# GuanLab/seekmer

Hardware: AMD Instinct MI355X
Metric: paired reads/sec mapped+quantified (higher is better)
Workload: dtype u64+f64; 1 GPU; configs[1]: synthetic ~190k-tx index (stand-in for ENSEMBL GRCh38 cDNA), 10000000 2x100bp synthetic pairs per GPU, map+classes+EM to the reference stop rule; transcripts=190402, kmer_slots=134217728, units_per_gpu=10000000, read_len=100, paired=True, classes=851072, class_map_rows=4208693, parallelism=reads sharded x1, RCCL all-reduce f64[T] per EM step, rccl_ranks=0

## Files before the change

include/seekmer_hip.h:

```cpp
#ifndef SEEKMER_HIP_H
#define SEEKMER_HIP_H

#include <stddef.h>
#include <stdint.h>

#ifdef __cplusplus
extern "C" {
#endif

#define SKM_OK 0
#define SKM_ERR_ARG 1
#define SKM_ERR_HIP 2
#define SKM_ERR_NO_DEVICE 3
#define SKM_ERR_COLLISION 4
#define SKM_ERR_STATE 5
#define SKM_ERR_IO 6
#define SKM_ERR_UNDEFINED 7
#define SKM_ERR_COMM 8

#define SKM_KMER_SIZE 25
#define SKM_MAX_FRAGMENT_LENGTH 2000


const char *skm_last_error(void);
// ... 194 lines not shown
                               int64_t n_tx, double *out);
int skm_effective_lengths_weights(int device, int64_t n, const double *p, const double *lengths,
                                  int64_t n_tx, double *out);

int skm_bias_correct(skm_index *index, int strand, const int64_t *observed, const double *tpm, const double *eff,
                     int64_t n_tx, double *expected_out, double *b_out, double *eff_out);
int skm_bias_correct_many(skm_index *index, int strand, int64_t n, const int64_t *observed, const double *tpm,
                          const double *eff, int64_t n_tx, double *expected_out, double *b_out, double *eff_out);
int skm_bias_fixed_weights(const double *tpm, const int32_t *windows, int64_t n_tx, uint64_t *limbs_out,
                           double *total_out);

typedef struct skm_quant skm_quant;
int skm_quant_create(int device, int64_t n_tx, int64_t n_classes,
                     const int64_t *class_offsets, const int32_t *class_targets,
                     const double *class_counts, skm_quant **out);
int skm_quant_create_from_mapper(skm_mapper *mapper, int64_t n_tx, skm_quant **out);
int skm_quant_destroy(skm_quant *quant);
int skm_quant_em(skm_quant *quant, double *x, const double *l, double rel_tol,
                 double x_floor, int64_t max_iters, int64_t fixed_iters,
                 int64_t *iters);
int skm_quant_bootstrap(skm_quant *quant, int64_t n_boot, uint64_t seed,
                        const double *x0, const double *l, double rel_tol,
                        double x_floor, int64_t max_iters, double *out,
                        int64_t *counts_out, int64_t *iters_out);
int skm_quant_bootstrap_tpm(skm_quant *quant, int64_t n_boot, uint64_t seed,
                            const double *x0, const double *l, double rel_tol,
                            double x_floor, int64_t max_iters, double *out,
                            int64_t *iters_out);
int skm_quant_bootstrap_share_tpm(skm_quant *quant, int64_t n_boot, int64_t first, int64_t step,
                                  uint64_t seed, const double *x0, const double *l, double rel_tol,
                                  double x_floor, int64_t max_iters, double *out,
                                  int64_t *iters_out);
int skm_quant_set_counts(skm_quant *quant, const double *class_counts);
int skm_quant_em_many(skm_quant *quant, int64_t n_sets, const double *counts, const double *x0,
                      const double *l, double rel_tol, double x_floor, int tpm, double *out,
                      int64_t *iters_out);
int skm_quant_em_blend(skm_quant *quant, int64_t n_cells, const int32_t *class_cell,
                       const double *weight, const double *cell_total, const double *x0,
                       const double *l, double rel_tol, double x_floor, int tpm, double *out,
                       int64_t *iters_out, double *counts_out);
int skm_quant_em_tables(int device, int64_t n_tx, int64_t n_tables, const int64_t *table_class_offsets,
                        const int64_t *class_offsets, const int32_t *class_targets,
                        const double *class_counts, const double *x0, const double *l, double rel_tol,
                        double x_floor, int64_t max_iters, int tpm, double *out, int64_t *iters);
int skm_set_quant_groups(int64_t n_tables, int64_t n_tx, const int64_t *table_classes,
                         const int64_t *table_ids, int64_t max_slots, int64_t *n_groups,
                         int64_t *group_first);
int skm_sample_set_quantify(skm_sample_set *set, const double *lengths, int64_t n_tx, double rel_tol,
                            double x_floor, int64_t max_iters, int64_t cap_samples,
                            int64_t *n_samples, double *tpm, double *effective_lengths,
                            int64_t *iters);
int skm_quant_components(skm_quant *quant, int64_t info[8], int32_t *tx_label, int32_t *tx_tile,
                         int32_t *class_tile);
int skm_quant_timing(skm_quant *quant, double timing[4]);

typedef struct skm_comm skm_comm;
int skm_comm_unique_id(void *id128);
int skm_comm_create(int device, const void *id128, int rank, int world, skm_comm **out);
int skm_comm_count(skm_comm *comm, int *count);
int skm_comm_destroy(skm_comm *comm);
int skm_mapper_exchange_tables(skm_mapper *send, int send_to, skm_mapper *recv, int recv_from, skm_comm *comm);
int skm_quant_set_comm(skm_quant *quant, skm_comm *comm);

int skm_quant_infer(skm_mapper *mapper, skm_comm *comm, const double *lengths, int64_t n_tx,
                    double rel_tol, double x_floor, int64_t max_iters,
                    double *tpm, double *effective_lengths, int64_t *iters);


typedef struct skm_built skm_built;
int skm_build_index(const char *pool, const int64_t *seq_offsets, int64_t n_seqs,
                    int n_threads, skm_built **out);
int skm_built_sizes(const skm_built *b, int64_t sizes[4]);
int skm_built_copy(const skm_built *b, void *kmers, void *contigs,
                   char *sequences, void *targets);
int skm_built_free(skm_built *b);

typedef struct skm_fastq skm_fastq;
int skm_fastq_open(const char *const *paths, int n_paths, int paired,
                   int64_t batch_units, skm_fastq **out);
int skm_fastq_set_allocator(skm_fastq *reader, void *(*alloc)(size_t), void (*release)(void *));
int skm_fastq_set_parallel(skm_fastq *reader, int n_threads, int *enabled);
int skm_fastq_set_shard(skm_fastq *reader, int rank, int world);
int skm_fastq_batch_index(const skm_fastq *reader, int64_t *index);
int skm_fastq_batch_read_length(const skm_fastq *reader, int64_t *read_len);
int skm_fastq_next(skm_fastq *reader, int64_t *n_units, const char **bases,
                   const int64_t **offsets, const char **names,
                   const int64_t **name_offsets);
typedef struct skm_fastq_slab skm_fastq_slab;
int skm_fastq_detach(skm_fastq *reader, skm_fastq_slab **slab);
int skm_fastq_recycle(skm_fastq *reader, skm_fastq_slab *slab);
int skm_fastq_close(skm_fastq *reader);

int skm_fastq_cache_bytes(int64_t bytes);
int skm_fastq_wait_unmapped(void);
typedef struct skm_fastq_prefault skm_fastq_prefault;
int skm_fastq_prefault_start(const char *const *paths, int n_paths, int n_threads, skm_fastq_prefault **out);
int skm_fastq_prefault_finish(skm_fastq_prefault *handle);

typedef struct skm_fastq_packed skm_fastq_packed;
int skm_fastq_packed_open(const char *const *paths, int n_paths, int paired, int n_threads,
                          int64_t chunk_bytes, int want_names, skm_fastq_packed **out);
int skm_fastq_packed_open_ranges(const char *const *paths, int n_paths, int paired, int n_threads,
                                 int64_t chunk_bytes, int want_names, const int64_t *begin,
                                 const int64_t *end, int64_t first_unit, skm_fastq_packed **out);
int skm_fastq_count_newlines(const char *path, int64_t chunk_bytes, int64_t first_chunk,
                             int64_t chunk_step, int n_threads, int64_t *counts, int64_t n_chunks,
// ... 35 lines not shown
```

seekmer_amd/_native.py:

```python
import ctypes
import os

_HERE = os.path.dirname(os.path.abspath(__file__))
HIP_LIB_PATH = os.environ.get('SKM_HIP_LIB') or os.path.join(_HERE, 'libseekmer_hip.so')
HOST_LIB_PATH = os.path.join(_HERE, 'libseekmer_host.so')

SKM_OK = 0
SKM_ERR_ARG = 1
SKM_ERR_HIP = 2
SKM_ERR_NO_DEVICE = 3
SKM_ERR_COLLISION = 4
SKM_ERR_STATE = 5
SKM_ERR_IO = 6
SKM_ERR_UNDEFINED = 7
SKM_ERR_COMM = 8

SKM_STRAND_NONE = 0
SKM_STRAND_FR = 1
SKM_STRAND_RF = 2

c_void_pp = ctypes.POINTER(ctypes.c_void_p)
c_i64p = ctypes.POINTER(ctypes.c_int64)
c_i32p = ctypes.POINTER(ctypes.c_int32)
c_f64p = ctypes.POINTER(ctypes.c_double)
# ... 115 lines not shown
                                       c_i64p]),
    'skm_sample_set_plan': (ctypes.c_int, [c_i64, c_i32p, c_i64p, c_i64, c_i64, c_i64p, c_i64p, c_i64p, c_i32p]),
    'skm_sample_set_split': (ctypes.c_int, [c_i64, c_i64p, c_i64p, c_i32p, c_i64, c_i64, c_i64p, c_i32p, c_i64p, c_i64p,
                                            c_i64p]),
    'skm_gene_sums': (ctypes.c_int, [ctypes.c_int, c_i64, c_i64, c_i64, c_i32p, c_f64p, c_f64p]),
    'skm_gene_unique_counts': (ctypes.c_int, [ctypes.c_int, c_i64, c_i64p, c_i32p, c_i64p, c_i32p, c_i64, c_i64, c_i64,
                                              c_i32p, c_i64p, c_i64p]),
    'skm_mapper_gene_counts': (ctypes.c_int, [ctypes.c_void_p, c_i64, c_i64, c_i32p, c_i64p, c_i64p]),
    'skm_sample_set_gene_counts': (ctypes.c_int, [ctypes.c_void_p, c_i64, c_i64, c_i32p, c_i64, c_i64p, c_i64p]),
    'skm_sample_set_gene_matrix': (ctypes.c_int, [ctypes.c_void_p, c_i64, c_i64, c_i32p, c_void_pp]),
    'skm_gene_matrix_from_classes': (ctypes.c_int, [ctypes.c_int, c_i64, c_i64p, c_i32p, c_i64p, c_i32p, c_i64, c_i64, c_i64,
                                                    c_i32p, c_void_pp]),
    'skm_gene_matrix_shape': (ctypes.c_int, [ctypes.c_void_p, c_i64p, c_i64p, c_i64p]),
    'skm_gene_matrix_read': (ctypes.c_int, [ctypes.c_void_p, c_i64p, c_i32p, c_i64p, c_i64p]),
    'skm_gene_matrix_destroy': (ctypes.c_int, [ctypes.c_void_p]),
    'skm_barcodes_create':(ctypes.c_int, [ctypes.c_int, ctypes.c_char_p, c_i64, ctypes.c_int, c_void_pp]),
    'skm_barcodes_destroy': (ctypes.c_int, [ctypes.c_void_p]),
    'skm_barcodes_assign': (ctypes.c_int, [ctypes.c_void_p, ctypes.POINTER(PackedReads), ctypes.c_int, ctypes.c_int,
                                           c_i32p, c_i64p, c_i64p]),
    'skm_units_group': (ctypes.c_int, [ctypes.c_int, c_i32p, c_i64, c_i64, c_i32p, c_i64p]),
    'skm_barcode_census_create': (ctypes.c_int, [ctypes.c_int, ctypes.c_int, c_void_pp]),
    'skm_barcode_census_destroy': (ctypes.c_int, [ctypes.c_void_p]),
    'skm_barcode_census_add': (ctypes.c_int, [ctypes.c_void_p, ctypes.POINTER(PackedReads), ctypes.c_int, c_i64p]),
    'skm_barcode_census_size': (ctypes.c_int, [ctypes.c_void_p, c_i64p, c_i64p]),
    'skm_barcode_census_ranked': (ctypes.c_int, [ctypes.c_void_p, c_i64, c_u64p, c_i64p]),
    'skm_barcode_census_pick': (ctypes.c_int, [ctypes.c_void_p, c_i64, ctypes.c_int, c_i64, c_u64p, c_i64p, c_i64p]),
    'skm_quant_create': (ctypes.c_int, [ctypes.c_int, c_i64, c_i64, c_i64p, c_i32p, c_f64p,
                                        c_void_pp]),
    'skm_quant_create_from_mapper': (ctypes.c_int, [ctypes.c_void_p, c_i64, c_void_pp]),
    'skm_quant_destroy': (ctypes.c_int, [ctypes.c_void_p]),
    'skm_quant_em': (ctypes.c_int, [ctypes.c_void_p, c_f64p, c_f64p, ctypes.c_double,
                                    ctypes.c_double, c_i64, c_i64, c_i64p]),
    'skm_quant_bootstrap': (ctypes.c_int, [ctypes.c_void_p, c_i64, ctypes.c_uint64, c_f64p,
                                           c_f64p, ctypes.c_double, ctypes.c_double, c_i64,
                                           c_f64p, c_i64p, c_i64p]),
    'skm_quant_bootstrap_tpm': (ctypes.c_int, [ctypes.c_void_p, c_i64, ctypes.c_uint64, c_f64p,
                                               c_f64p, ctypes.c_double, ctypes.c_double, c_i64,
                                               c_f64p, c_i64p]),
    'skm_quant_bootstrap_share_tpm': (ctypes.c_int, [ctypes.c_void_p, c_i64, c_i64, c_i64, ctypes.c_uint64, c_f64p,
                                                     c_f64p, ctypes.c_double, ctypes.c_double, c_i64,
                                                     c_f64p, c_i64p]),
    'skm_quant_set_counts': (ctypes.c_int, [ctypes.c_void_p, c_f64p]),
    'skm_quant_em_many': (ctypes.c_int, [ctypes.c_void_p, c_i64, c_f64p, c_f64p, c_f64p, ctypes.c_double,
                                         ctypes.c_double, ctypes.c_int, c_f64p, c_i64p]),
    'skm_quant_em_blend': (ctypes.c_int, [ctypes.c_void_p, c_i64, c_i32p, c_f64p, c_f64p, c_f64p, c_f64p,
                                          ctypes.c_double, ctypes.c_double, ctypes.c_int, c_f64p, c_i64p, c_f64p]),
    'skm_quant_em_tables': (ctypes.c_int, [ctypes.c_int, c_i64, c_i64, c_i64p, c_i64p, c_i32p, c_f64p, c_f64p, c_f64p,
                                           ctypes.c_double, ctypes.c_double, c_i64, ctypes.c_int, c_f64p, c_i64p]),
    'skm_set_quant_groups': (ctypes.c_int, [c_i64, c_i64, c_i64p, c_i64p, c_i64, c_i64p, c_i64p]),
    'skm_sample_set_quantify': (ctypes.c_int, [ctypes.c_void_p, c_f64p, c_i64, ctypes.c_double, ctypes.c_double, c_i64,
                                               c_i64, c_i64p, c_f64p, c_f64p, c_i64p]),
    'skm_quant_timing': (ctypes.c_int, [ctypes.c_void_p, c_f64p]),
    'skm_quant_components': (ctypes.c_int, [ctypes.c_void_p, c_i64p, c_i32p, c_i32p, c_i32p]),
    'skm_comm_unique_id': (ctypes.c_int, [ctypes.c_void_p]),
    'skm_comm_create': (ctypes.c_int, [ctypes.c_int, ctypes.c_void_p, ctypes.c_int, ctypes.c_int,
                                       c_void_pp]),
    'skm_comm_count': (ctypes.c_int, [ctypes.c_void_p, ctypes.POINTER(ctypes.c_int)]),
    'skm_comm_destroy': (ctypes.c_int, [ctypes.c_void_p]),
    'skm_mapper_exchange_tables': (ctypes.c_int, [ctypes.c_void_p, ctypes.c_int, ctypes.c_void_p, ctypes.c_int,
                                                  ctypes.c_void_p]),
    'skm_quant_set_comm': (ctypes.c_int, [ctypes.c_void_p, ctypes.c_void_p]),
    'skm_quant_infer': (ctypes.c_int, [ctypes.c_void_p, ctypes.c_void_p, c_f64p, c_i64, ctypes.c_double,
                                       ctypes.c_double, c_i64, c_f64p, c_f64p, c_i64p]),
}

HOST_SYMBOLS = {
    'skm_build_index': (ctypes.c_int, [ctypes.c_void_p, c_i64p, c_i64, ctypes.c_int, c_void_pp]),
    'skm_built_sizes': (ctypes.c_int, [ctypes.c_void_p, c_i64p]),
    'skm_built_copy': (ctypes.c_int, [ctypes.c_void_p, ctypes.c_void_p, ctypes.c_void_p,
                                      ctypes.c_void_p, ctypes.c_void_p]),
    'skm_built_free': (ctypes.c_int, [ctypes.c_void_p]),
    'skm_fastq_open': (ctypes.c_int, [ctypes.POINTER(ctypes.c_char_p), ctypes.c_int, ctypes.c_int,
                                      c_i64, c_void_pp]),
    'skm_fastq_set_allocator': (ctypes.c_int, [ctypes.c_void_p, ctypes.c_void_p, ctypes.c_void_p]),
    'skm_fastq_set_parallel': (ctypes.c_int, [ctypes.c_void_p, ctypes.c_int, ctypes.POINTER(ctypes.c_int)]),
    'skm_fastq_set_shard': (ctypes.c_int, [ctypes.c_void_p, ctypes.c_int, ctypes.c_int]),
    'skm_fastq_batch_read_length': (ctypes.c_int, [ctypes.c_void_p, c_i64p]),
    'skm_fastq_batch_index': (ctypes.c_int, [ctypes.c_void_p, c_i64p]),
    'skm_fastq_next': (ctypes.c_int, [ctypes.c_void_p, c_i64p, c_void_pp, c_void_pp, c_void_pp,
                                      c_void_pp]),
    'skm_fastq_detach': (ctypes.c_int, [ctypes.c_void_p, c_void_pp]),
    'skm_fastq_recycle': (ctypes.c_int, [ctypes.c_void_p, ctypes.c_void_p]),
    'skm_fastq_close': (ctypes.c_int, [ctypes.c_void_p]),
    'skm_fastq_cache_bytes': (ctypes.c_int, [c_i64]),
    'skm_fastq_wait_unmapped': (ctypes.c_int, []),
    'skm_fastq_packed_open': (ctypes.c_int, [ctypes.POINTER(ctypes.c_char_p), ctypes.c_int, ctypes.c_int,
                                             ctypes.c_int, c_i64, ctypes.c_int, c_void_pp]),
    'skm_fastq_packed_open_ranges': (ctypes.c_int, [ctypes.POINTER(ctypes.c_char_p), ctypes.c_int, ctypes.c_int,
                                                    ctypes.c_int, c_i64, ctypes.c_int, c_i64p, c_i64p, c_i64, c_void_pp]),
    'skm_fastq_count_newlines': (ctypes.c_int, [ctypes.c_char_p, c_i64, c_i64, c_i64, ctypes.c_int, c_i64p, c_i64,
                                                ctypes.POINTER(ctypes.c_int)]),
    'skm_fastq_locate_line': (ctypes.c_int, [ctypes.c_char_p, c_i64, c_i64p, c_i64, c_i64, c_i64p]),
    'skm_fastq_packed_set_allocator': (ctypes.c_int, [ctypes.c_void_p, ctypes.c_void_p, ctypes.c_void_p]),
    'skm_fastq_packed_next': (ctypes.c_int, [ctypes.c_void_p, ctypes.POINTER(PackedReads)]),
    'skm_fastq_packed_stats': (ctypes.c_int, [ctypes.c_void_p, c_i64p]),
    'skm_fastq_prefault_start': (ctypes.c_int, [ctypes.POINTER(ctypes.c_char_p), ctypes.c_int, ctypes.c_int, c_void_pp]),
    'skm_fastq_prefault_finish': (ctypes.c_int, [ctypes.c_void_p]),
    'skm_fastq_packed_estimate': (ctypes.c_int, [ctypes.c_void_p, c_i64p]),
    'skm_fastq_packed_close': (ctypes.c_int, [ctypes.c_void_p]),
    'skm_pack_reads': (ctypes.c_int, [ctypes.c_void_p, c_i64p, c_i64, ctypes.c_int32, ctypes.c_void_p,
                                      ctypes.c_void_p, ctypes.c_void_p, ctypes.c_void_p, c_i64, c_i64p,
                                      ctypes.c_int]),
    'skm_pack_set_variant': (ctypes.c_int, [ctypes.c_int]),
    'skm_packed_gather': (ctypes.c_int, [ctypes.POINTER(PackedReads), c_i64, c_i32p, c_i64, ctypes.c_int32,
                                         ctypes.c_void_p, ctypes.c_void_p, ctypes.c_void_p, ctypes.c_void_p, c_i64,
                                         c_i64p]),
# ... 81 lines not shown
```

seekmer_amd/csrc/skm_abi_quant.hip:

```cpp
#include "skm_abi_samples.h"

#include <dlfcn.h>
#include <algorithm>
#include <chrono>
#include <cstdio>
#include <cstdlib>
#include <cstring>
#include <functional>
#include <memory>
#include <mutex>
#include <vector>

using namespace skm;
using namespace skm::abi;

struct skm_quant {
    ~skm_quant()
    {
        (void)hipSetDevice(device);
        if (stream) (void)hipStreamSynchronize(stream);
    }
    int device = 0;
    PoolStream stream;
    PoolTimingEvent ev[2];
// ... 657 lines not shown
    lap("destroy");
    return SKM_OK;
}

extern "C" int skm_quant_destroy(skm_quant *q)
{
    if (!q) return SKM_OK;
    STALE_CHECK("quant_destroy entry");
    delete q;
    STALE_CHECK("quant_destroy exit");
    return SKM_OK;
}

extern "C" int skm_quant_em(skm_quant *q, double *x, const double *l, double rel_tol, double x_floor,
                            int64_t max_iters, int64_t fixed_iters, int64_t *iters)
{
    if (!q || !x || !l) return fail(SKM_ERR_ARG, "NULL argument");
    std::lock_guard<std::mutex> lock(q->mu);
    SKM_TRY(set_device(q->device));
    HIP_TRY(hipMemcpyAsync(q->x0.p, x, q->n_tx * 8, hipMemcpyHostToDevice, q->stream));
    HIP_TRY(hipMemcpyAsync(q->eff_len.p, l, q->n_tx * 8, hipMemcpyHostToDevice, q->stream));
    int64_t it = 0;
    SKM_TRY(em_run(q, rel_tol, x_floor, max_iters, fixed_iters, &it));
    HIP_TRY(hipMemcpy(x, (it & 1) ? q->x1.p : q->x0.p, q->n_tx * 8, hipMemcpyDeviceToHost));
    if (iters) *iters = it;
    return SKM_OK;
}

extern "C" int skm_quant_components(skm_quant *q, int64_t info[8], int32_t *tx_label, int32_t *tx_tile,
                                    int32_t *class_tile)
{
    if (!q || !info) return fail(SKM_ERR_ARG, "NULL argument");
    std::lock_guard<std::mutex> lock(q->mu);
    SKM_TRY(set_device(q->device));
    const auto &t = q->tiles;
    info[0] = t.built ? 1 : 0;
    info[1] = t.n_tiles;
    info[2] = t.n_oversize;
    info[3] = em_uses_tiles(q) ? 1 : 0;
    info[4] = EM_TILE_PAIRS; info[5] = EM_TILE_CLASSES; info[6] = EM_TILE_TX; info[7] = EM_TILE_SEGMENT;
    if (!t.built) {
        if (tx_label || tx_tile || class_tile) return fail(SKM_ERR_ARG, "no component tiles were built for this handle");
        return SKM_OK;
    }
    HIP_TRY(hipStreamSynchronize(q->stream));
    if (tx_label) HIP_TRY(hipMemcpy(tx_label, t.tx_label.p, q->n_tx * 4, hipMemcpyDeviceToHost));
    if (tx_tile) HIP_TRY(hipMemcpy(tx_tile, t.tx_tile.p, q->n_tx * 4, hipMemcpyDeviceToHost));
    if (class_tile && q->n_classes) {
        std::vector<int32_t> tile(q->n_classes), perm(q->n_classes);
        HIP_TRY(hipMemcpy(tile.data(), t.cls_tile.p, q->n_classes * 4, hipMemcpyDeviceToHost));
        HIP_TRY(hipMemcpy(perm.data(), q->perm.p, q->n_classes * 4, hipMemcpyDeviceToHost));
        for (int64_t k = 0; k < q->n_classes; ++k) class_tile[perm[k]] = tile[k];
    }
    return SKM_OK;
}

extern "C" int skm_quant_set_counts(skm_quant *q, const double *class_counts)
{
    if (!q || (!class_counts && q->n_classes)) return fail(SKM_ERR_ARG, "NULL argument");
    std::lock_guard<std::mutex> lock(q->mu);
    SKM_TRY(set_device(q->device));
    const double total = np_sum_host(class_counts, q->n_classes);
    if (q->n_classes) {
        SKM_TRY(q->cls_count_saved.ensure(q->n_classes));
        HIP_TRY(hipMemcpyAsync(q->cls_count_saved.p, class_counts, q->n_classes * 8, hipMemcpyHostToDevice, q->stream));
        launch_permute_f64(q->cls_count_saved.p, q->perm.p, q->n_classes, q->cls_count.p, false, q->stream);
        HIP_TRY(hipGetLastError());
        HIP_TRY(hipStreamSynchronize(q->stream));
    }
    q->n_total = total;
    return SKM_OK;
}

namespace {

template <class Fill>
int em_group_run(skm_quant *q, int64_t n_problems, Fill &&fill, bool batched, int64_t slot_cap, const double *x0,
                 const double *l, double rel_tol, double x_floor, int64_t max_iters, double *out, int64_t *iters_out,
                 bool tpm)
{
    const int64_t C = q->n_classes, T = q->n_tx;
    skm_quant::Batch &w = q->batch;
    const int64_t group = std::max<int64_t>(1, std::min<int64_t>(n_problems, (int64_t)(1LL << 28) / T));
    const int64_t by_counts = std::max<int64_t>(1, (int64_t)((1LL << 31) / (8 * std::max<int64_t>(C, 1))));
    int64_t slots = batched ? std::max<int64_t>(1, std::min(group, by_counts)) : 1;
    if (slot_cap > 0) slots = std::min(slots, slot_cap);
    SKM_TRY(q->cls_count_saved.ensure(C));
    SKM_TRY(q->x_start.ensure(T));
    SKM_TRY(q->boot_out.ensure((size_t)(slots * T)));
    SKM_TRY(w.totals.ensure((size_t)(2 * slots)));
    HIP_TRY(hipMemcpyAsync(q->cls_count_saved.p, q->cls_count.p, C * 8, hipMemcpyDeviceToDevice, q->stream));
    HIP_TRY(hipMemcpyAsync(q->eff_len.p, l, T * 8, hipMemcpyHostToDevice, q->stream));
    HIP_TRY(hipMemcpyAsync(q->x_start.p, x0, T * 8, hipMemcpyHostToDevice, q->stream));
    const double saved_total = q->n_total;
    int rc = SKM_OK;
    DBuf<double> sums;
    auto restore = on_exit([&]() {
        (void)hipMemcpyAsync(q->cls_count.p, q->cls_count_saved.p, C * 8, hipMemcpyDeviceToDevice, q->stream);
        (void)hipStreamSynchronize(q->stream);
        q->n_total = saved_total;
    });
    auto problem_checked = [&](int64_t b, int64_t *it_out, double *dst) -> int {
        SKM_TRY(fill(b, (int64_t)1, q->cls_count.p, w.totals.p));
        HIP_TRY(hipGetLastError());
        double total = 0.0;
        HIP_TRY(hipMemcpyAsync(&total, w.totals.p, 8, hipMemcpyDeviceToHost, q->stream));
// ... 801 lines not shown
```

seekmer_amd/csrc/skm_em.hip:

```cpp
#include "skm_em_core.h"

namespace skm {

__device__ bool em_evaluate(const EmProblem &p, int n_parts, int64_t steps_done, bool publish);

struct EmWholeTable {
    const EmProblem &p;
    __device__ __forceinline__ int64_t cls_first() const { return 0; }
    __device__ __forceinline__ int64_t cls_end() const { return p.n_classes; }
    __device__ __forceinline__ int64_t row_first() const { return 0; }
    __device__ __forceinline__ int64_t row_end() const { return p.n_rows; }
    __device__ __forceinline__ double n_total() const { return p.n_total; }
    __device__ __forceinline__ bool done() const { return p.ctl[CTL_DONE] != 0; }
    __device__ __forceinline__ bool judge(int eval_parts, int64_t steps_done) const { return em_evaluate(p, eval_parts, steps_done, true); }
    __device__ __forceinline__ int64_t part() const { return blockIdx.x; }
};

__global__ void __launch_bounds__(256)
em_inner_kernel(EmProblem p, int parity, int eval_parts, int64_t steps_done)
{
    em_inner_body(p, EmWholeTable{p}, parity, eval_parts > 0 && blockIdx.x == 0, eval_parts, steps_done, blockIdx.x * (int64_t)blockDim.x + threadIdx.x,
                  (int64_t)gridDim.x * blockDim.x);
}

// ... 44 lines not shown
        em_note_change(v, x_old[t], p.x_floor, local_max, flags);
    }
    if (em_block_reduce<1>(local_max, flags)) {
        p.part_max[blockIdx.x] = local_max;
        p.part_flags[blockIdx.x] = flags;
    }
}

__device__ bool em_evaluate(const EmProblem &p, int n_parts, int64_t steps_done, bool publish)
{
    __shared__ int s_done;
    double m = 0.0;
    unsigned int f = 0;
    for (int b = threadIdx.x; b < n_parts; b += blockDim.x) {
        const double o = p.part_max[b];
        m = o > m ? o : m;
        f |= p.part_flags[b];
    }
    if (p.n_extra > 0) {
        const int64_t first = (steps_done - 1 - p.extra_first) * p.n_extra;
        for (int64_t b = threadIdx.x; b < p.n_extra; b += blockDim.x) {
            const double o = p.extra_max[first + b];
            m = o > m ? o : m;
            f |= p.extra_flags[first + b];
        }
    }
    if (em_block_reduce<1>(m, f)) {
        const EmVerdict verdict = em_stop_rule(f, m, p.rel_tol, steps_done, p.max_iters, p.fixed_iters);
        if (publish) {
            if (verdict.undefined) p.ctl[CTL_UNDEFINED] = 1;
            p.ctl[CTL_ITERS] = (unsigned long long)steps_done;
            p.ctl[CTL_DONE] = verdict.done ? 1ULL : 0ULL;
        }
        s_done = verdict.done ? 1 : 0;
    }
    __syncthreads();
    return s_done != 0;
}

__global__ void __launch_bounds__(256)
em_decide_kernel(EmProblem p, int n_parts, int64_t steps_done)
{
    if (p.ctl[CTL_DONE]) return;
    em_evaluate(p, n_parts, steps_done, true);
}

#ifndef SKM_EM_TILE_EXPERIMENT
#define SKM_EM_TILE_EXPERIMENT 0
#endif
#ifndef SKM_EM_CLASS_BATCH
#define SKM_EM_CLASS_BATCH 4
#endif
constexpr int EM_CLASS_BATCH = SKM_EM_CLASS_BATCH;
static_assert(EM_CLASS_BATCH == EM_TILE_CLASS_BATCH || EM_CLASS_BATCH == 1, "the set-up orders classes by turns of this width");

__device__ __forceinline__ unsigned long long em_tile_arrive(unsigned long long *judge, bool has, double m, unsigned int f)
{
    if (has) {
        unsigned long long *word_max = judge + EM_JUDGE_MAX + threadIdx.x, *word_flags = judge + EM_JUDGE_FLAGS + threadIdx.x;
        const unsigned long long bits = (unsigned long long)__double_as_longlong(m);
        if (__hip_atomic_load(word_max, __ATOMIC_RELAXED, __HIP_MEMORY_SCOPE_AGENT) < bits)
            __hip_atomic_fetch_max(word_max, bits, __ATOMIC_RELAXED, __HIP_MEMORY_SCOPE_AGENT);
        if (f & ~(unsigned int)__hip_atomic_load(word_flags, __ATOMIC_RELAXED, __HIP_MEMORY_SCOPE_AGENT))
            __hip_atomic_fetch_or(word_flags, (unsigned long long)f, __ATOMIC_RELAXED, __HIP_MEMORY_SCOPE_AGENT);
    }
    asm volatile("s_waitcnt vmcnt(0)" ::: "memory");
    unsigned long long arrived = 0;
    if (threadIdx.x == 0)
        arrived = __hip_atomic_fetch_add(judge + EM_JUDGE_ARRIVED, 1ULL, __ATOMIC_RELAXED, __HIP_MEMORY_SCOPE_AGENT) + 1ULL;
    return __shfl(arrived, 0, 64);
}
__device__ __forceinline__ void em_tiles_judge(const EmProblem &p, unsigned long long *judge, bool has, int64_t first_step, int n_steps)
{
    double m = 0.0;
    unsigned int f = 0;
    if (has) {
        m = __longlong_as_double((long long)__hip_atomic_exchange(judge + EM_JUDGE_MAX + threadIdx.x, 0ULL, __ATOMIC_RELAXED,
                                                                 __HIP_MEMORY_SCOPE_AGENT));
        f = (unsigned int)__hip_atomic_exchange(judge + EM_JUDGE_FLAGS + threadIdx.x, 0ULL, __ATOMIC_RELAXED, __HIP_MEMORY_SCOPE_AGENT);
    }
    if (threadIdx.x == 0) __hip_atomic_store(judge + EM_JUDGE_ARRIVED, 0ULL, __ATOMIC_RELAXED, __HIP_MEMORY_SCOPE_AGENT);
    bool undefined = false, done = false;
    int64_t steps_done = first_step;
    for (int s = 0; s < n_steps && !done; ++s) {
        steps_done = first_step + s + 1;
        const EmVerdict verdict = em_stop_rule(__shfl(f, s, 64), __shfl(m, s, 64), p.rel_tol, steps_done, p.max_iters, p.fixed_iters);
        undefined |= verdict.undefined;
        done = verdict.done;
    }
    if (threadIdx.x != 0) return;
    if (undefined) p.ctl[CTL_UNDEFINED] = 1;
    p.ctl[CTL_ITERS] = (unsigned long long)steps_done;
    p.ctl[CTL_DONE] = done ? 1ULL : 0ULL;
}

__global__ void __launch_bounds__(256)
em_local_chunk_kernel(EmProblem p, EmTiles tl, const double *x_in, int n_steps, int64_t first_step)
{
    static_assert(EM_TILE_TX <= 8 * 32, "a lane group of the row phase takes at most eight transcripts");
    __shared__ double s_x[2][EM_TILE_TX];
    __shared__ double s_eff[EM_TILE_TX];
    __shared__ double s_inner[EM_TILE_CLASSES];
    __shared__ double s_count[EM_TILE_CLASSES];
    __shared__ double s_max[EM_CHUNK_MAX][4];
    __shared__ unsigned int s_flags[EM_CHUNK_MAX][4];
    __shared__ int32_t s_tx[EM_TILE_TX];
    __shared__ uint16_t s_cls_tx[EM_TILE_PAIRS], s_tx_cls[EM_TILE_PAIRS];
    __shared__ uint16_t s_cls_off[EM_TILE_CLASSES + 1], s_tx_off[EM_TILE_TX + 1];
    const int64_t tile = tl.order ? tl.order[tl.order_reversed ? tl.n_tiles - 1 - blockIdx.x : blockIdx.x] : blockIdx.x;
    const int64_t tx0 = tl.tile_tx[tile], cls0 = tl.tile_cls[tile];
    const int n_tx = (int)(tl.tile_tx[tile + 1] - tx0), n_cls = (int)(tl.tile_cls[tile + 1] - cls0);
    const int64_t cp0 = tl.cls_pair[cls0], tp0 = tl.tx_pair[tx0];
    const int n_pairs = (int)(tl.cls_pair[cls0 + n_cls] - cp0);
    if (n_tx > EM_TILE_TX || n_cls > EM_TILE_CLASSES || n_pairs > EM_TILE_PAIRS || n_tx < 0 || n_cls < 0 || n_pairs < 0) {
        if (threadIdx.x == 0) { p.ctl[CTL_TILE_FAULT] = 1; p.ctl[CTL_DONE] = 1; }
        return;
    }
    const int tid = threadIdx.x;
    if (p.ctl[CTL_DONE]) {
        const int64_t steps = (int64_t)p.ctl[CTL_ITERS], at = steps - 1 - (first_step - n_steps);
        if (p.ctl[CTL_TILE_FAULT] || first_step < n_steps || at < 0 || at >= n_steps) return;
        const double *__restrict__ from = tl.snap + at * p.n_tx;
        double *__restrict__ to = p.x[steps & 1];
        for (int i = tid; i < n_tx; i += 256) {
            const int32_t t = tl.tx_list[tx0 + i];
            to[t] = from[t];
        }
        return;
    }
    for (int j = tid; j < n_pairs; j += 256) {
        s_cls_tx[j] = tl.cls_tx[cp0 + j];
        s_tx_cls[j] = tl.tx_cls[tp0 + j];
    }
    for (int k = tid; k <= n_cls; k += 256) {
        s_cls_off[k] = (uint16_t)(tl.cls_pair[cls0 + k] - cp0);
        if (k < n_cls) s_count[k] = p.cls_count[tl.cls_list[cls0 + k]];
        if ((SKM_EM_TILE_EXPERIMENT & 1) && k < n_cls) s_inner[k] = 1.0;
    }
    for (int i = tid; i <= n_tx; i += 256) {
        s_tx_off[i] = (uint16_t)(tl.tx_pair[tx0 + i] - tp0);
        if (i < n_tx) {
            const int32_t t = tl.tx_list[tx0 + i];
            s_tx[i] = t;
            s_x[0][i] = x_in[t];
            s_eff[i] = p.eff_len[t];
        }
    }
    __syncthreads();
    const int sub = tid & 7, wave = tid >> 6;
    for (int step = 0; step < n_steps; ++step) {
        const double *x = s_x[step & 1];
        double *x_new = s_x[(step & 1) ^ 1];
        if (!(SKM_EM_TILE_EXPERIMENT & 1)) {
            for (int k = tid; k < n_cls; k += 256) {
                const int end = s_cls_off[k + 1];
                double s = 0.0;
                if (EM_CLASS_BATCH == 1) {
                    for (int j = s_cls_off[k]; j < end; ++j) s += x[s_cls_tx[j]];
                } else {
                    for (int j = s_cls_off[k]; j < end; j += EM_CLASS_BATCH) {
                        int t[EM_CLASS_BATCH];
                        double v[EM_CLASS_BATCH];
#pragma unroll
                        for (int b = 0; b < EM_CLASS_BATCH; ++b) t[b] = s_cls_tx[min(j + b, end - 1)];
#pragma unroll
                        for (int b = 0; b < EM_CLASS_BATCH; ++b) v[b] = x[t[b]];
                        s += v[0];
#pragma unroll
                        for (int b = 1; b < EM_CLASS_BATCH; ++b) {
                            const double with = s + v[b];
                            s = j + b < end ? with : s;
                        }
                    }
                }
                s_inner[k] = s / s_count[k];
            }
        }
        __syncthreads();
        double local_max = 0.0;
        unsigned int flags = 0;
        double my_a = 0.0, my_xt = 0.0;
        int my_i = -1, turn = 0;
        if (!(SKM_EM_TILE_EXPERIMENT & 2)) {
            for (int i = tid >> 3; i < n_tx; i += 32, ++turn) {
                const double xt = x[i];
                const int end = s_tx_off[i + 1];
                int begin = s_tx_off[i];
                double a = 0.0;
                do {
                    const int row_end = min(begin + EM_ROW_CAP, end);
                    a += em_row_sum<false>(s_tx_cls, s_inner, begin, row_end, sub, xt);
                    begin = row_end;
                } while (begin < end);
                if (turn == sub) { my_a = a; my_xt = xt; my_i = i; }
            }
        }
        if (my_i >= 0) {
            const double v = em_new_abundance(my_a, s_eff[my_i], p.n_total);
            x_new[my_i] = v;
            tl.snap[step * p.n_tx + s_tx[my_i]] = v;
            em_note_change(v, my_xt, p.x_floor, local_max, flags);
        }
        em_wave_reduce<1>(local_max, flags);
        if ((tid & 63) == 0) { s_max[step][wave] = local_max; s_flags[step][wave] = flags; }
        __syncthreads();
    }
    if (tid >= 64) return;
    double m = 0.0;
    unsigned int f = 0;
    if (tid < n_steps) em_fold_waves(s_max[tid], s_flags[tid], 1, m, f);
    if (tl.judge == nullptr) {
        if (tid < n_steps) {
            tl.step_max[tid * tl.n_tiles + tile] = m;
            tl.step_flags[tid * tl.n_tiles + tile] = f;
        }
        return;
    }
    if (em_tile_arrive(tl.judge, tid < n_steps, m, f) != (unsigned long long)tl.n_tiles) return;
    em_tiles_judge(p, tl.judge, tid < n_steps, first_step, n_steps);
}

#if SKM_EM_JUDGE_LAUNCH
__global__ void __launch_bounds__(64 * EM_CHUNK_MAX)
em_local_decide_kernel(EmProblem p, EmTiles tl, int64_t first_step, int n_steps)
{
    if (p.ctl[CTL_DONE]) return;
    __shared__ double s_max[EM_CHUNK_MAX];
    __shared__ unsigned int s_flags[EM_CHUNK_MAX];
    const int step = threadIdx.x >> 6, lane = threadIdx.x & 63;
    if (step < n_steps) {
        double m = 0.0;
        unsigned int f = 0;
        const double *__restrict__ step_max = tl.step_max + step * tl.n_tiles;
        const unsigned int *__restrict__ step_flags = tl.step_flags + step * tl.n_tiles;
        int64_t b = lane;
        for (; b + 7 * 64 < tl.n_tiles; b += 8 * 64) {
            double o[8];
            unsigned int g[8];
#pragma unroll
            for (int k = 0; k < 8; ++k) { o[k] = step_max[b + 64 * k]; g[k] = step_flags[b + 64 * k]; }
#pragma unroll
            for (int k = 0; k < 8; ++k) { m = o[k] > m ? o[k] : m; f |= g[k]; }
        }
        for (; b < tl.n_tiles; b += 64) {
            const double o = step_max[b];
            m = o > m ? o : m;
            f |= step_flags[b];
        }
// ... 671 lines not shown
```

seekmer_amd/csrc/skm_em_core.h:

```cpp
#pragma once
#include "skm_kernels.h"

namespace skm {

template <int STRIDE>
__device__ __forceinline__ double em_tuple_sum(const int32_t *__restrict__ ids, int64_t begin, int64_t end,
                                               const double *__restrict__ x, int at)
{
    double s = 0.0;
    int64_t j = begin;
    for (; j + 4 <= end; j += 4) {
        const int32_t t0 = ids[j], t1 = ids[j + 1], t2 = ids[j + 2], t3 = ids[j + 3];
        const double x0 = x[(int64_t)t0 * STRIDE + at], x1 = x[(int64_t)t1 * STRIDE + at];
        const double x2 = x[(int64_t)t2 * STRIDE + at], x3 = x[(int64_t)t3 * STRIDE + at];
        s += x0; s += x1; s += x2; s += x3;
    }
    for (; j < end; ++j) s += x[(int64_t)ids[j] * STRIDE + at];
    return s;
}

__device__ __forceinline__ double em_row_butterfly(double s)
{
    s += __shfl_xor(s, 4, 8);
    s += __shfl_xor(s, 2, 8);
    s += __shfl_xor(s, 1, 8);
    return s;
}

template <bool PAIRED, typename Cls, typename Off>
__device__ __forceinline__ double em_row_sum(const Cls *tx_cls, const double *inner, Off begin, Off end, int sub, double xt)
{
    double s = 0.0;
    Off e = begin + sub;
    if (PAIRED) {
        for (; e + 8 < end; e += 16) {
            const Cls c0 = tx_cls[e], c1 = tx_cls[e + 8];
            const double i0 = inner[c0], i1 = inner[c1];
            s += xt / i0;
            s += xt / i1;
        }
    }
    for (; e < end; e += 8) s += xt / inner[tx_cls[e]];
    return em_row_butterfly(s);
}

template <int R>
__device__ __forceinline__ void em_row_sums(const int32_t *__restrict__ tx_cls, const double *__restrict__ inner_all,
                                            int64_t begin, int64_t end, int sub, const double *__restrict__ xt,
                                            double (&xr)[R], double (&s)[R])
{
#pragma unroll
    for (int r = 0; r < R; ++r) { xr[r] = xt[r]; s[r] = 0.0; }
    for (int64_t e = begin + sub; e < end; e += 8) {
        const double *__restrict__ inner = inner_all + (int64_t)tx_cls[e] * R;
#pragma unroll
        for (int r = 0; r < R; ++r) s[r] += xr[r] / inner[r];
    }
#pragma unroll
    for (int r = 0; r < R; ++r) s[r] = em_row_butterfly(s[r]);
}

__device__ __forceinline__ unsigned int em_row_publish(double *row_sum, int64_t slot, double s, unsigned int *arrivals_t, bool counts)
{
    __hip_atomic_store(reinterpret_cast<unsigned long long *>(row_sum) + slot, (unsigned long long)__double_as_longlong(s),
                       __ATOMIC_RELAXED, __HIP_MEMORY_SCOPE_AGENT);
    asm volatile("s_waitcnt vmcnt(0)" ::: "memory");
    return counts ? atomicAdd(arrivals_t, 1u) + 1u : 0u;
}
__device__ __forceinline__ double em_row_published(const double *row_sum, int64_t slot)
{
    return __longlong_as_double((long long)__hip_atomic_load(reinterpret_cast<const unsigned long long *>(row_sum) + slot,
                                                             __ATOMIC_RELAXED, __HIP_MEMORY_SCOPE_AGENT));
}
template <int STRIDE>
__device__ __forceinline__ double em_rows_published_sum(const double *row_sum, int64_t first_row, int64_t rows_of_t, int sub)
{
    double a = 0.0;
    if (STRIDE == 1) {
        for (int64_t k0 = 0; k0 < rows_of_t; k0 += 8) {
            const int64_t k = k0 + sub;
            const double mine = k < rows_of_t ? em_row_published(row_sum, first_row + k) : 0.0;
#pragma unroll
            for (int j = 0; j < 8; ++j) {
                const double v = __shfl(mine, j, 8);
                if (k0 + j < rows_of_t) a += v;
            }
        }
    } else {
        for (int64_t k = 0; k < rows_of_t; ++k) a += em_row_published(row_sum, (first_row + k) * STRIDE + sub);
    }
    return a;
}
__device__ __forceinline__ void em_row_arrivals_reset(unsigned int *arrivals_t) { atomicExch(arrivals_t, 0u); }

template <int STRIDE>
__device__ __forceinline__ double em_rows_stored_sum(const double *__restrict__ row_sum, int64_t first, int64_t end, int at)
{
    double a = 0.0;
    for (int64_t r = first; r < end; ++r) a += row_sum[r * STRIDE + at];
    return a;
}

__device__ __forceinline__ double em_new_abundance(double a, double eff, double n_total)
{
    double v = a / eff / n_total;
    if (v != v) v = 0.0;
    return v;
}
__device__ __forceinline__ void em_note_change(double v, double before, double x_floor, double &local_max, unsigned int &flags)
{
    if (v > x_floor) {
        const double change = fabs(v - before) / v;
        if (change != change) flags |= 2u;
        else if (change > local_max) local_max = change;
        flags |= 1u;
    }
}

template <int LOWEST>
__device__ __forceinline__ void em_wave_reduce(double &m, unsigned int &f)
{
    for (int d = 32; d >= LOWEST; d >>= 1) {
        const double o = __shfl_xor(m, d, 64);
        m = o > m ? o : m;
        f |= __shfl_xor(f, d, 64);
    }
}
__device__ __forceinline__ void em_fold_waves(const double *s_max, const unsigned int *s_flags, int stride, double &m, unsigned int &f)
{
    m = s_max[0];
    f = s_flags[0];
    for (int w = 1; w < 4; ++w) { m = s_max[w * stride] > m ? s_max[w * stride] : m; f |= s_flags[w * stride]; }
}
template <int LOWEST>
__device__ __forceinline__ bool em_block_reduce(double &m, unsigned int &f)
{
    __shared__ double s_max[4][LOWEST];
    __shared__ unsigned int s_flags[4][LOWEST];
    em_wave_reduce<LOWEST>(m, f);
    const int wave = threadIdx.x >> 6, r = threadIdx.x & (LOWEST - 1);
    if ((threadIdx.x & 63) < LOWEST) { s_max[wave][r] = m; s_flags[wave][r] = f; }
    __syncthreads();
    if (threadIdx.x >= LOWEST) return false;
    em_fold_waves(&s_max[0][r], &s_flags[0][r], LOWEST, m, f);
    return true;
}

struct EmVerdict { bool done, undefined; };
__device__ __forceinline__ EmVerdict em_stop_rule(unsigned int f, double m, double rel_tol, int64_t steps_done,
                                                  int64_t max_iters, int64_t fixed_iters)
{
    if (fixed_iters > 0) return {steps_done >= fixed_iters, false};
    if (!(f & 1u)) return {true, true};
    bool done = (f & 2u) || !(m > rel_tol);
    if (max_iters > 0 && steps_done >= max_iters) done = true;
    return {done, false};
}


template <class Problem, class View>
__device__ __forceinline__ void em_inner_body(const Problem &p, const View &v, int parity, bool judges, int eval_parts,
                                              int64_t steps_done, int64_t lane, int64_t lanes)
{
    const int64_t cls_end = v.cls_end();
    const int64_t c_first = v.cls_first() + lane;
    int64_t begin_first = 0, end_first = 0;
    double count_first = 1.0;
    if (c_first < cls_end) {
        begin_first = p.cls_offset[c_first];
        end_first = p.cls_offset[c_first + 1];
        count_first = p.cls_count[c_first];
    }
    if (judges) {
        if (v.done()) return;
        if (v.judge(eval_parts, steps_done)) return;
    } else if (v.done()) {
        return;
    }
    const double *__restrict__ x = p.x[parity];
// ... 58 lines not shown
```

seekmer_amd/csrc/skm_kernels.h:

```cpp
#pragma once
#include "skm_device.h"

namespace skm {

struct MapBatch {
    const uint32_t *records;
    int64_t n_units;
    int32_t words_per_read;
    int32_t record_words;
    int32_t paired;
    int32_t *workspace;
    int32_t *rec_unit;
    uint64_t *rec_key;
    unsigned long long *rec_tuple;
    int32_t keep_spans;
    int32_t *unit_begin, *unit_end;
    Coord *unit_anchor;
    int32_t *unit_entries;
    int64_t ids_capacity;
    int32_t ids_chunk;
    unsigned long long *ids_cursor;
    unsigned long long *fld;
    unsigned long long *stats;
    int32_t vote[8];
// ... 168 lines not shown
    const double *cls_count;
    double *inner;
    const int64_t *row_start;
    const int32_t *row_tx;
    const int32_t *tx_cls;
    const int64_t *tx_row;
    double *row_sum;
    const double *eff_len;
    double *x[2];
    double *acc;
    double n_total;
    double rel_tol, x_floor;
    unsigned long long *ctl;
    double *part_max;
    unsigned int *part_flags;
    int64_t max_iters, fixed_iters;
    int fused;
    unsigned int *arrivals;
    const double *extra_max;
    const unsigned int *extra_flags;
    int64_t n_extra, extra_first;
};
enum { CTL_DONE = 0, CTL_ITERS = 1, CTL_UNDEFINED = 3, CTL_TILE_FAULT = 4 };
#ifndef SKM_EM_FINAL_BLOCKS
#define SKM_EM_FINAL_BLOCKS 2048
#endif
constexpr int EM_FINAL_BLOCKS = SKM_EM_FINAL_BLOCKS;
void launch_em_inner(const EmProblem &p, int parity, bool judge_previous, int64_t steps_done, hipStream_t stream);
void launch_em_decide(const EmProblem &p, int64_t steps_done, hipStream_t stream);
void launch_em_rows(const EmProblem &p, int parity, hipStream_t stream);
void launch_em_rows_finalize(const EmProblem &p, int parity, hipStream_t stream);
void launch_em_rows_acc(const EmProblem &p, int parity, hipStream_t stream);
void launch_em_rows_to_acc(const EmProblem &p, hipStream_t stream);
void launch_em_finalize(const EmProblem &p, int parity, bool from_acc, hipStream_t stream);
void launch_em_result(const unsigned long long *ctl, const double *x0, const double *x1, int64_t n, double *out,
                      hipStream_t stream);

#ifndef SKM_EM_TILE_PAIRS
#define SKM_EM_TILE_PAIRS 2048
#endif
#ifndef SKM_EM_TILE_CLASSES
#define SKM_EM_TILE_CLASSES 512
#endif
#ifndef SKM_EM_TILE_TX
#define SKM_EM_TILE_TX 128
#endif
#ifndef SKM_EM_TILE_SEGMENT
#define SKM_EM_TILE_SEGMENT 256
#endif
constexpr int EM_TILE_PAIRS = SKM_EM_TILE_PAIRS, EM_TILE_CLASSES = SKM_EM_TILE_CLASSES, EM_TILE_TX = SKM_EM_TILE_TX;
static_assert(EM_TILE_PAIRS <= 65535 && EM_TILE_CLASSES <= 65535 && EM_TILE_TX <= 65535, "tile-local indices and offsets are 16 bits wide");
constexpr int EM_TILE_SEGMENT = SKM_EM_TILE_SEGMENT;
static_assert(EM_TILE_SEGMENT > 0, "a packing run holds at least one transcript id");
constexpr int EM_CHUNK_MAX = 16;
constexpr int EM_TILE_CLASS_BATCH = 4;
struct EmTiles {
    int64_t n_tiles;
    const int64_t *tile_tx;
    const int64_t *tile_cls;
    const int32_t *tx_list;
    const int32_t *cls_list;
    const int64_t *cls_pair;
    const int64_t *tx_pair;
    const uint16_t *cls_tx;
    const uint16_t *tx_cls;
    double *step_max;
    unsigned int *step_flags;
    double *snap;
    const int32_t *order;
    int32_t order_reversed;
    unsigned long long *judge;
};
enum { EM_JUDGE_MAX = 0, EM_JUDGE_FLAGS = 16, EM_JUDGE_ARRIVED = 32, EM_JUDGE_WORDS = 48 };
static_assert(EM_CHUNK_MAX <= 16, "a step's word of each kind");
constexpr int EM_CTL_WORDS = 16;
#ifndef SKM_EM_JUDGE_LAUNCH
#define SKM_EM_JUDGE_LAUNCH 0
#endif
void launch_em_local_chunk(const EmProblem &p, const EmTiles &tiles, const double *x_in, int n_steps, int64_t first_step,
                           hipStream_t stream);
#if SKM_EM_JUDGE_LAUNCH
void launch_em_local_decide(const EmProblem &p, const EmTiles &tiles, int64_t first_step, int n_steps, hipStream_t stream);
#endif

constexpr int EM_BATCH = 8;
struct EmBatchProblem {
    int64_t n_tx, n_classes, n_rows;
    const int64_t *cls_offset;
    const int32_t *ids;
    const int64_t *row_start;
    const int32_t *row_tx;
    const int32_t *tx_cls;
    const int64_t *tx_row;
    const double *eff_len;
    const double *cls_count;
    double *inner;
    double *row_sum;
    double *x[2];
    double *place_total;
    double rel_tol, x_floor;
    unsigned long long *ctl;
    double *part_max;
    unsigned int *part_flags;
    int managed;
    unsigned long long *mgr;
    int64_t *iters_out;
// ... 265 lines not shown
```

Before: 1.071 billion pairs/s.

## Add optional precomputed quotient array in EM tiles and DPP lane reductions

Behind a build flag, the EM tile kernel can precompute each pair's x/inner quotient into a shared array, in batches, and then sum transcript rows from it. The same flag allows an optional dense lane-per-transcript finalize. Separately, the 8-lane row butterfly and the low strides of the wave reduction now use DPP moves instead of shuffles, which is meant to cut LDS-routed cross-lane traffic. The quotient path is off by default; the DPP change always applies. A geometry query ABI is also added.

```diff
diff --git a/include/seekmer_hip.h b/include/seekmer_hip.h
--- a/include/seekmer_hip.h
+++ b/include/seekmer_hip.h
@@ -270,6 +270,7 @@
                             int64_t *iters);
 int skm_quant_components(skm_quant *quant, int64_t info[8], int32_t *tx_label, int32_t *tx_tile,
                          int32_t *class_tile);
+int skm_em_tile_geometry(int64_t info[8]);
 int skm_quant_timing(skm_quant *quant, double timing[4]);
 
 typedef struct skm_comm skm_comm;
diff --git a/seekmer_amd/_native.py b/seekmer_amd/_native.py
--- a/seekmer_amd/_native.py
+++ b/seekmer_amd/_native.py
@@ -191,6 +191,7 @@
                                                c_i64, c_i64p, c_f64p, c_f64p, c_i64p]),
     'skm_quant_timing': (ctypes.c_int, [ctypes.c_void_p, c_f64p]),
     'skm_quant_components': (ctypes.c_int, [ctypes.c_void_p, c_i64p, c_i32p, c_i32p, c_i32p]),
+    'skm_em_tile_geometry': (ctypes.c_int, [c_i64p]),
     'skm_comm_unique_id': (ctypes.c_int, [ctypes.c_void_p]),
     'skm_comm_create': (ctypes.c_int, [ctypes.c_int, ctypes.c_void_p, ctypes.c_int, ctypes.c_int,
                                        c_void_pp]),
diff --git a/seekmer_amd/csrc/skm_abi_quant.hip b/seekmer_amd/csrc/skm_abi_quant.hip
--- a/seekmer_amd/csrc/skm_abi_quant.hip
+++ b/seekmer_amd/csrc/skm_abi_quant.hip
@@ -733,6 +733,14 @@
         HIP_TRY(hipMemcpy(perm.data(), q->perm.p, q->n_classes * 4, hipMemcpyDeviceToHost));
         for (int64_t k = 0; k < q->n_classes; ++k) class_tile[perm[k]] = tile[k];
     }
+    return SKM_OK;
+}
+
+extern "C" int skm_em_tile_geometry(int64_t info[8])
+{
+    if (!info) return fail(SKM_ERR_ARG, "NULL argument");
+    info[0] = EM_TILE_PAIRS; info[1] = EM_TILE_CLASSES; info[2] = EM_TILE_TX; info[3] = EM_TILE_SEGMENT;
+    info[4] = EM_TILE_QUOT; info[5] = EM_TILE_BATCHES; info[6] = EM_ROW_CAP; info[7] = EM_CHUNK_MAX;
     return SKM_OK;
 }
 
diff --git a/seekmer_amd/csrc/skm_em.hip b/seekmer_amd/csrc/skm_em.hip
--- a/seekmer_amd/csrc/skm_em.hip
+++ b/seekmer_amd/csrc/skm_em.hip
@@ -120,6 +120,10 @@
 #define SKM_EM_CLASS_BATCH 4
 #endif
 constexpr int EM_CLASS_BATCH = SKM_EM_CLASS_BATCH;
+#ifndef SKM_EM_TILE_DENSE_FINALIZE
+#define SKM_EM_TILE_DENSE_FINALIZE 0
+#endif
+static_assert(EM_TILE_QUOT > 0 || !SKM_EM_TILE_DENSE_FINALIZE, "the lane-per-transcript finalize belongs to the quotient array's build");
 static_assert(EM_CLASS_BATCH == EM_TILE_CLASS_BATCH || EM_CLASS_BATCH == 1, "the set-up orders classes by turns of this width");
 
 __device__ __forceinline__ unsigned long long em_tile_arrive(unsigned long long *judge, bool has, double m, unsigned int f)
@@ -175,6 +179,13 @@
     __shared__ int32_t s_tx[EM_TILE_TX];
     __shared__ uint16_t s_cls_tx[EM_TILE_PAIRS], s_tx_cls[EM_TILE_PAIRS];
     __shared__ uint16_t s_cls_off[EM_TILE_CLASSES + 1], s_tx_off[EM_TILE_TX + 1];
+#if SKM_EM_TILE_QUOT
+    static_assert(EM_TILE_TX <= 256, "a pair's tile-local transcript is one byte");
+    __shared__ uint8_t s_pair_tx[EM_TILE_PAIRS];
+    __shared__ double s_quot[EM_TILE_QUOT];
+    __shared__ uint16_t s_batch_end[EM_TILE_BATCHES];
+    __shared__ int s_n_batches;
+#endif
     const int64_t tile = tl.order ? tl.order[tl.order_reversed ? tl.n_tiles - 1 - blockIdx.x : blockIdx.x] : blockIdx.x;
     const int64_t tx0 = tl.tile_tx[tile], cls0 = tl.tile_cls[tile];
     const int n_tx = (int)(tl.tile_tx[tile + 1] - tx0), n_cls = (int)(tl.tile_cls[tile + 1] - cls0);
@@ -216,6 +227,34 @@
     }
     __syncthreads();
     const int sub = tid & 7, wave = tid >> 6;
+#if SKM_EM_TILE_QUOT
+    const int group = tid >> 3;
+    for (int i = group; i < n_tx; i += 32)
+        for (int e = s_tx_off[i] + sub; e < s_tx_off[i + 1]; e += 8) s_pair_tx[e] = (uint8_t)i;
+    if constexpr (EM_TILE_BATCHES > 1) {
+        if (tid < 64) {
+            int first = 0, n = 0;
+            while (first < n_tx && n >= 0) {
+                const int base = s_tx_off[first];
+                int fit = 0;
+                for (int i0 = 0; i0 <= n_tx; i0 += 64) {
+                    const int i = i0 + tid;
+                    fit += __popcll(__ballot(i > first && i <= n_tx && (int)s_tx_off[i] - base <= EM_TILE_QUOT));
+                }
+                first += fit;
+                if (fit == 0 || n == EM_TILE_BATCHES) n = -1;
+                else { if (tid == 0) s_batch_end[n] = (uint16_t)first; ++n; }
+            }
+            if (tid == 0) s_n_batches = n;
+        }
+        __syncthreads();
+        if (s_n_batches < 0) {
+            if (tid == 0) { p.ctl[CTL_TILE_FAULT] = 1; p.ctl[CTL_DONE] = 1; }
+            return;
+        }
+    }
+    const int n_batches = EM_TILE_BATCHES > 1 ? s_n_batches : 1;
+#endif
     for (int step = 0; step < n_steps; ++step) {
         const double *x = s_x[step & 1];
         double *x_new = s_x[(step & 1) ^ 1];
@@ -248,8 +287,10 @@
         double local_max = 0.0;
         unsigned int flags = 0;
         double my_a = 0.0, my_xt = 0.0;
-        int my_i = -1, turn = 0;
+        int my_i = -1;
         if (!(SKM_EM_TILE_EXPERIMENT & 2)) {
+#if !SKM_EM_TILE_QUOT
+            int turn = 0;
             for (int i = tid >> 3; i < n_tx; i += 32, ++turn) {
                 const double xt = x[i];
                 const int end = s_tx_off[i + 1];
@@ -262,6 +303,36 @@
                 } while (begin < end);
                 if (turn == sub) { my_a = a; my_xt = xt; my_i = i; }
             }
+#else
+            for (int b = 0, first = 0; b < n_batches; ++b) {
+                const int last = EM_TILE_BATCHES > 1 ? (int)s_batch_end[b] : n_tx;
+                const int base = s_tx_off[first], top = s_tx_off[last];
+                for (int j = base + tid; j < top; j += 256) s_quot[j - base] = x[s_pair_tx[j]] / s_inner[s_tx_cls[j]];
+                __syncthreads();
+                int turn = first > group ? (first - group + 31) >> 5 : 0;
+                for (int i = group + 32 * turn; i < last; i += 32, ++turn) {
+                    const int end = s_tx_off[i + 1] - base;
+                    int begin = s_tx_off[i] - base;
+                    double a = 0.0;
+                    do {
+                        const int row_end = min(begin + EM_ROW_CAP, end);
+                        a += em_row_sum_of<false>(begin, row_end, sub, [&](int e) { return s_quot[e]; });
+                        begin = row_end;
+                    } while (begin < end);
+#if SKM_EM_TILE_DENSE_FINALIZE
+                    if (sub == 0) x_new[i] = a;
+#else
+                    if (turn == sub) { my_a = a; my_xt = x[i]; my_i = i; }
+#endif
+                }
+                first = last;
+                if (b + 1 < n_batches) __syncthreads();
+            }
+#endif
+#if SKM_EM_TILE_DENSE_FINALIZE
+            __syncthreads();
+            if (tid < n_tx) { my_a = x_new[tid]; my_xt = x[tid]; my_i = tid; }
+#endif
         }
         if (my_i >= 0) {
             const double v = em_new_abundance(my_a, s_eff[my_i], p.n_total);
diff --git a/seekmer_amd/csrc/skm_em_core.h b/seekmer_amd/csrc/skm_em_core.h
--- a/seekmer_amd/csrc/skm_em_core.h
+++ b/seekmer_amd/csrc/skm_em_core.h
@@ -19,29 +19,51 @@
     return s;
 }
 
+template <int D>
+__device__ __forceinline__ int em_from_lane_xor(int v)
+{
+    static_assert(D == 1 || D == 2 || D == 4 || D == 8, "a partner inside the row of 16 lanes");
+    if constexpr (D == 1) return __builtin_amdgcn_update_dpp(v, v, 0xB1, 0xF, 0xF, false);
+    if constexpr (D == 2) return __builtin_amdgcn_update_dpp(v, v, 0x4E, 0xF, 0xF, false);
+    if constexpr (D == 8) return __builtin_amdgcn_update_dpp(v, v, 0x128, 0xF, 0xF, false);
+    if constexpr (D == 4) {
+        const int up = __builtin_amdgcn_update_dpp(v, v, 0x104, 0xF, 0x5, false);
+        return __builtin_amdgcn_update_dpp(up, v, 0x114, 0xF, 0xA, false);
+    }
+}
+template <int D>
+__device__ __forceinline__ double em_from_lane_xor(double v)
+{
+    return __hiloint2double(em_from_lane_xor<D>(__double2hiint(v)), em_from_lane_xor<D>(__double2loint(v)));
+}
+
 __device__ __forceinline__ double em_row_butterfly(double s)
 {
-    s += __shfl_xor(s, 4, 8);
-    s += __shfl_xor(s, 2, 8);
-    s += __shfl_xor(s, 1, 8);
+    s += em_from_lane_xor<4>(s);
+    s += em_from_lane_xor<2>(s);
+    s += em_from_lane_xor<1>(s);
     return s;
 }
 
-template <bool PAIRED, typename Cls, typename Off>
-__device__ __forceinline__ double em_row_sum(const Cls *tx_cls, const double *inner, Off begin, Off end, int sub, double xt)
+template <bool PAIRED, typename Off, typename Term>
+__device__ __forceinline__ double em_row_sum_of(Off begin, Off end, int sub, Term term)
 {
     double s = 0.0;
     Off e = begin + sub;
     if (PAIRED) {
         for (; e + 8 < end; e += 16) {
-            const Cls c0 = tx_cls[e], c1 = tx_cls[e + 8];
-            const double i0 = inner[c0], i1 = inner[c1];
-            s += xt / i0;
-            s += xt / i1;
-        }
-    }
-    for (; e < end; e += 8) s += xt / inner[tx_cls[e]];
+            const double t0 = term(e), t1 = term((Off)(e + 8));
+            s += t0;
+            s += t1;
+        }
+    }
+    for (; e < end; e += 8) s += term(e);
     return em_row_butterfly(s);
+}
+template <bool PAIRED, typename Cls, typename Off>
+__device__ __forceinline__ double em_row_sum(const Cls *tx_cls, const double *inner, Off begin, Off end, int sub, double xt)
+{
+    return em_row_sum_of<PAIRED>(begin, end, sub, [&](Off e) { return xt / inner[tx_cls[e]]; });
 }
 
 template <int R>
@@ -117,14 +139,27 @@
     }
 }
 
+template <int D, int LOWEST>
+__device__ __forceinline__ void em_wave_reduce_step(double &m, unsigned int &f)
+{
+    if constexpr (D >= LOWEST) {
+        const double o = em_from_lane_xor<D>(m);
+        m = o > m ? o : m;
+        f |= (unsigned int)em_from_lane_xor<D>((int)f);
+    }
+}
 template <int LOWEST>
 __device__ __forceinline__ void em_wave_reduce(double &m, unsigned int &f)
 {
-    for (int d = 32; d >= LOWEST; d >>= 1) {
+    for (int d = 32; d >= LOWEST && d >= 16; d >>= 1) {
         const double o = __shfl_xor(m, d, 64);
         m = o > m ? o : m;
         f |= __shfl_xor(f, d, 64);
     }
+    em_wave_reduce_step<8, LOWEST>(m, f);
+    em_wave_reduce_step<4, LOWEST>(m, f);
+    em_wave_reduce_step<2, LOWEST>(m, f);
+    em_wave_reduce_step<1, LOWEST>(m, f);
 }
 __device__ __forceinline__ void em_fold_waves(const double *s_max, const unsigned int *s_flags, int stride, double &m, unsigned int &f)
 {
diff --git a/seekmer_amd/csrc/skm_kernels.h b/seekmer_amd/csrc/skm_kernels.h
--- a/seekmer_amd/csrc/skm_kernels.h
+++ b/seekmer_amd/csrc/skm_kernels.h
@@ -244,6 +244,14 @@
 static_assert(EM_TILE_PAIRS <= 65535 && EM_TILE_CLASSES <= 65535 && EM_TILE_TX <= 65535, "tile-local indices and offsets are 16 bits wide");
 constexpr int EM_TILE_SEGMENT = SKM_EM_TILE_SEGMENT;
 static_assert(EM_TILE_SEGMENT > 0, "a packing run holds at least one transcript id");
+#ifndef SKM_EM_TILE_QUOT
+#define SKM_EM_TILE_QUOT 0
+#endif
+constexpr int EM_TILE_QUOT = SKM_EM_TILE_QUOT;
+static_assert(EM_TILE_QUOT == 0 ||
+              (EM_TILE_QUOT >= (EM_TILE_CLASSES < EM_TILE_PAIRS ? EM_TILE_CLASSES : EM_TILE_PAIRS) && EM_TILE_QUOT <= EM_TILE_PAIRS),
+              "a batch of quotients holds the pairs of any one transcript of a tile");
+constexpr int EM_TILE_BATCHES = EM_TILE_QUOT == 0 || EM_TILE_QUOT >= EM_TILE_PAIRS ? 1 : 2 * ((EM_TILE_PAIRS + EM_TILE_QUOT - 1) / EM_TILE_QUOT) + 1;
 constexpr int EM_CHUNK_MAX = 16;
 constexpr int EM_TILE_CLASS_BATCH = 4;
 struct EmTiles {
```

Result: no change. 1.063 billion pairs/s (-0.7%).
